# microsoft/StemGNN

Hardware: AMD Instinct MI355X
Metric: forecast-steps/sec (train) (higher is better)
Workload: dtype f32

## Files before the change

stemgnn_amd/csrc/gru.hip:

```cpp
#include <hip/hip_runtime.h>

#include "../../include/stemgnn_hip.h"
#include "gemm2.h"
#include "wgrad.h"
#include "dq_reduce.h"
#include "gemm_core.h"
#include "gru_wide.h"

#define SG_TRY(e)                                \
  do {                                           \
    hipError_t _e = (e);                         \
    if (_e != hipSuccess) return -(int)_e;       \
  } while (0)

__device__ __forceinline__ float gru_sigmoid(float v) { return 1.f / (1.f + expf(-v)); }
__device__ __forceinline__ int gru_uniform(int v) { return __builtin_amdgcn_readfirstlane(v); }

struct GruGiOp {
  const float *x, *w_ih, *b_ih;
  float* gi;
  int B, S, Hd, W;
  unsigned *za, *zb;
  unsigned na, nb;
  __device__ bool setup(int, int& M, int& N, int& K0, int& K1) const {
// ... 465 lines not shown
typedef float gru_f2 __attribute__((ext_vector_type(2)));
#ifndef GRU_NR_FWD
#define GRU_NR_FWD 8
#endif
#ifndef GRU_NR_BWD
#define GRU_NR_BWD 16
#endif
#ifndef GRU_NR4
#define GRU_NR4 16
#endif
#define GRU_NR2(P, OW) (((OW) == 1 && (P) <= 4) ? GRU_NR_BWD : 64)
#define GRU_NR3(KU) ((KU) <= 58 ? GRU_NR_FWD : 32)
template <int KU, int NR>
struct GruBcast {
  static constexpr int NRK = NR < KU ? (NR & ~3) : ((KU + 3) & ~3);
  static constexpr int NL = NRK < KU ? (KU - NRK + 3) / 4 : 0;
  float4 v[NL > 0 ? NL : 1];
  float hv;
  __device__ __forceinline__ GruBcast(float hv_, float* lrow, int lane) : hv(hv_) {
    if constexpr (NL > 0) {
      lrow[lane] = hv_;
      asm volatile("" ::: "memory");
#pragma unroll
      for (int i = 0; i < NL; ++i) v[i] = *reinterpret_cast<const float4*>(lrow + NRK + 4 * i);
      __builtin_amdgcn_sched_barrier(0);
    }
  }
  __device__ __forceinline__ gru_f2 pair(int kk) const {
    if (kk < NRK) return gru_f2{gru_bcast(hv, kk), gru_bcast(hv, kk + 1)};
    const float4 t = v[NL > 0 ? (kk - NRK) >> 2 : 0];
    return ((kk - NRK) & 2) ? gru_f2{t.z, t.w} : gru_f2{t.x, t.y};
  }
};
template <int KU, int NR>
__device__ __forceinline__ float gru_matvec(const gru_f2 (&wr)[32], float hv, float* lrow, int lane) {
  const GruBcast<KU, NR> bc(hv, lrow, lane);
  gru_f2 a0 = {0.f, 0.f}, a1 = {0.f, 0.f};
#pragma unroll
  for (int kk = 0; kk + 3 < KU; kk += 4) {
    a0 = __builtin_elementwise_fma(wr[kk >> 1], bc.pair(kk), a0);
    a1 = __builtin_elementwise_fma(wr[(kk >> 1) + 1], bc.pair(kk + 2), a1);
  }
  if constexpr ((KU & 3) != 0) a0 = __builtin_elementwise_fma(wr[(KU - 2) >> 1], bc.pair(KU - 2), a0);
  return (a0.x + a1.x) + (a0.y + a1.y);
}
__device__ __forceinline__ float gru_poll_lane(const gru_u64* g, unsigned tag, bool active, int* status) {
  float v = 0.f;
  if (active) v = gru_consume(g, tag, status);
  return v;
}

#ifdef GRU_PROF
#define GRU_T(var) const long long var = (long long)__builtin_readcyclecounter()
#define GRU_ACC(acc, t1, t0) acc += (t1) - (t0)
#else
#define GRU_T(var)
#define GRU_ACC(acc, t1, t0)
#endif
template <int KU, int NR>
__device__ __forceinline__ void gru_matvec3(const gru_f2 (&w0)[32], const gru_f2 (&w1)[32], const gru_f2 (&w2)[32],
                                            float hv, float* lrow, int lane, float& o0, float& o1, float& o2) {
  const GruBcast<KU, NR> bc(hv, lrow, lane);
  gru_f2 a0 = {0.f, 0.f}, b0 = {0.f, 0.f}, a1 = {0.f, 0.f}, b1 = {0.f, 0.f}, a2 = {0.f, 0.f}, b2 = {0.f, 0.f};
#pragma unroll
  for (int kk = 0; kk + 3 < KU; kk += 4) {
    const gru_f2 h0 = bc.pair(kk), h1 = bc.pair(kk + 2);
    a0 = __builtin_elementwise_fma(w0[kk >> 1], h0, a0);
    a1 = __builtin_elementwise_fma(w1[kk >> 1], h0, a1);
    a2 = __builtin_elementwise_fma(w2[kk >> 1], h0, a2);
    b0 = __builtin_elementwise_fma(w0[(kk >> 1) + 1], h1, b0);
    b1 = __builtin_elementwise_fma(w1[(kk >> 1) + 1], h1, b1);
    b2 = __builtin_elementwise_fma(w2[(kk >> 1) + 1], h1, b2);
  }
  if constexpr ((KU & 3) != 0) {
    const gru_f2 h0 = bc.pair(KU - 2);
    a0 = __builtin_elementwise_fma(w0[(KU - 2) >> 1], h0, a0);
    a1 = __builtin_elementwise_fma(w1[(KU - 2) >> 1], h0, a1);
    a2 = __builtin_elementwise_fma(w2[(KU - 2) >> 1], h0, a2);
  }
  o0 = (a0.x + b0.x) + (a0.y + b0.y);
  o1 = (a1.x + b1.x) + (a1.y + b1.y);
  o2 = (a2.x + b2.x) + (a2.y + b2.y);
}
template <int P, int KU, int OW>
__global__ __launch_bounds__(3 * (P / OW) * 64) void gru_bwd_cluster2_kernel(const float* __restrict__ dout, const float* __restrict__ w_hh,
                                                                      const float* __restrict__ h_all,
                                                                      const float* __restrict__ reserve, int B, int S, int Hd,
                                                                      gru_u64* __restrict__ xbuf, int* __restrict__ status,
                                                                      float* __restrict__ dgi, float* __restrict__ dghn,
                                                                      int s_hi, int s_lo, float* __restrict__ carry,
                                                                      int s_mark, unsigned* __restrict__ progress,
                                                                      gru_u64* __restrict__ xid, int allow_fast) {
  static_assert(P % OW == 0, "owners per wave");
  constexpr int NTH = 3 * (P / OW) * 64;
  __shared__ float part[2][3 * P][64];
  __shared__ __attribute__((aligned(16))) float lrow[3 * P][64];
  __shared__ int s_fast;
  int b, p;
  gru_cluster_ids(B, P, b, p);
  if (b >= B) return;
  const bool fast = P > 1 && gru_same_xcd(xid + (size_t)b * P, p, P, allow_fast, status, &s_fast, threadIdx.x);
  const int U = (Hd + P - 1) / P;
  const int tid = threadIdx.x, lane = tid & 63;
  const int wave = gru_uniform(tid >> 6);
  const int g = wave / (P / OW), q0 = (wave - g * (P / OW)) * OW;
  const int u0 = p * U, un = max(0, min(Hd, u0 + U) - u0);
  const int H3 = 3 * Hd;
  gru_f2 wr[OW][32];
  int k0[OW], kn[OW];
#pragma unroll
  for (int o = 0; o < OW; ++o) {
    k0[o] = ((q0 + o + p) % P) * U;
    kn[o] = max(0, min(Hd, k0[o] + U) - k0[o]);
    const bool lane_ok = lane < un;
    const float* wcol = w_hh + ((size_t)g * Hd + (kn[o] > 0 ? k0[o] : 0)) * Hd + (lane_ok ? u0 + lane : 0);
#pragma unroll
    for (int kk = 0; kk < KU; ++kk) {
      const float v = wcol[(size_t)(kk < kn[o] ? kk : 0) * Hd];
      wr[o][kk >> 1][kk & 1] = (lane_ok && kk < kn[o]) ? v : 0.f;
    }
  }
  const int gu = u0 + (tid < un ? tid : 0);
  float dhz = s_hi < S - 1 ? carry[(size_t)b * Hd + gu] : 0.f;
  for (int i = tid; i < 2 * 3 * P * 64; i += NTH) (&part[0][0][0])[i] = 0.f;
  size_t prow = (size_t)s_hi * B + b;
  float p_do = dout[prow * Hd + gu];
  float p_r = reserve[prow * 4 * Hd + gu], p_z = reserve[prow * 4 * Hd + Hd + gu];
  float p_n = reserve[prow * 4 * Hd + 2 * Hd + gu], p_g = reserve[prow * 4 * Hd + 3 * Hd + gu];
  float p_h = h_all[(s_hi > 0 ? prow - B : prow) * Hd + gu];
  __syncthreads();

#ifdef GRU_PROF
  long long c_poll = 0, c_mv = 0, c_bar = 0, c_gate = 0;
#endif
  for (int s = s_hi; s >= s_lo; --s) {
    const size_t row = (size_t)s * B + b;
    const unsigned tag = (unsigned)(S - s);
    gru_u64* xb = xbuf + ((size_t)(tag & 1) * B + b) * H3;
    float own_dr = 0.f;
    GRU_T(t0);
    if (tid < un) {
      float dh = p_do + dhz;
#pragma unroll
      for (int w = 0; w < 3 * P; ++w) dh += part[(tag + 1) & 1][w][tid];
      const float r = p_r, z = p_z, n = p_n, ghn = p_g;
      const float hprev = s > 0 ? p_h : 0.f;
      const float dn = dh * (1.f - z) * (1.f - n * n);
      const float dz = dh * (hprev - n) * z * (1.f - z);
      const float dr = dn * ghn * r * (1.f - r);
      const float dnr = dn * r;
      own_dr = dr;
      dhz = dh * z;
      if (s > 0) {
        gru_publish_x(xb + gu, tag, dr, fast);
        gru_publish_x(xb + Hd + gu, tag, dz, fast);
        gru_publish_x(xb + 2 * Hd + gu, tag, dnr, fast);
        const size_t rn = row - B;
        p_do = dout[rn * Hd + gu];
        p_r = reserve[rn * 4 * Hd + gu]; p_z = reserve[rn * 4 * Hd + Hd + gu];
        p_n = reserve[rn * 4 * Hd + 2 * Hd + gu]; p_g = reserve[rn * 4 * Hd + 3 * Hd + gu];
        p_h = h_all[(s > 1 ? rn - B : rn) * Hd + gu];
      }
      float* go = dgi + row * H3;
      go[gu] = dr; go[Hd + gu] = dz; go[2 * Hd + gu] = dn;
      dghn[row * Hd + gu] = dnr;
    }
// ... 250 lines not shown
    gru_hh_gemms(q, base, base + (size_t)3 * S * B * Hd, base, base, base, Hd);
    p.hh_form = gru_hh_form(q, Hd).form;
  }
  return p;
}
extern "C" int stemgnn_gru_paths(int B, int S, int Hd, int W, int cus, int* out) {
  if (B <= 0 || S <= 0 || Hd <= 0 || W <= 0 || !out) return SG_EINVAL;
  const GruPlan p = gru_plan(B, S, Hd, W, cus > 0 ? gru_limit_of_cus(cus) : gru_resident_limit());
  const bool wide = p.fwd_family == SG_GRU_FAM_WIDE;
  out[SG_GRU_FWD_FAMILY] = p.fwd_family; out[SG_GRU_FWD_P] = p.PF; out[SG_GRU_FWD_K] = p.KF;
  out[SG_GRU_GI_STREAM] = p.gi_stream;
  out[SG_GRU_BWD_FAMILY] = p.bwd_family; out[SG_GRU_BWD_P] = p.P; out[SG_GRU_BWD_KU] = p.KU;
  out[SG_GRU_BWD_SLICES] = p.slices; out[SG_GRU_IH_FOLDED] = p.fold_ih; out[SG_GRU_HH_FORM] = p.hh_form;
  out[SG_GRU_IH_SLABS] = p.ih_sum; out[SG_GRU_RANK2_OK] = p.rank2_ok;
  out[SG_GRU_WIDE_PASSES] = wide ? (B + GW_BP - 1) / GW_BP : 0;
  out[SG_GRU_WIDE_MT] = wide ? p.wide.MT : 0;
  out[SG_GRU_WIDE_GWF] = wide ? gru_wide_gwf_class(p.wide) : 0;
  out[SG_GRU_WIDE_GWB] = wide ? gru_wide_gwb_class(p.wide) : 0;
  return 0;
}

extern "C" size_t stemgnn_gru_fwd_scratch_floats(int B, int S, int Hd) {
  return (size_t)3 * Hd * Hd + (size_t)3 * S * B * Hd + gru_xbuf_floats(B, Hd) + 4;
}
static size_t gru_bwd_scratch_base(int B, int S, int Hd, int W) {
  return (size_t)4 * S * B * Hd + (size_t)GRU_NSPLIT * 3 * Hd * (Hd + 1) + (size_t)gru_ih_slabs(B) * 3 * Hd * (W + 1) +
         gru_xbuf_floats(B, Hd) + 4 + (size_t)B * Hd + 8 + 136;
}
constexpr size_t GRU_OVL_CLAIMS = 64 * 33;
static size_t gru_ovl_words(int S) { return (((size_t)S + 4 + GRU_OVL_CLAIMS + 64 + 8) + 3) & ~(size_t)3; }
extern "C" size_t stemgnn_gru_bwd_scratch_floats(int B, int S, int Hd, int W) {
  return ((gru_bwd_scratch_base(B, S, Hd, W) + 3) & ~(size_t)3) + gru_ovl_words(S);
}
extern "C" size_t stemgnn_gru_bwd_ctl_words(int S) { return S > 0 ? gru_ovl_words(S) + 64 : 0; }

extern "C" int stemgnn_gru_bwd_cus(int B, int Hd) {
  if (B <= 0 || Hd <= 0) return 0;
  const GruPlan pl = gru_plan(B, Hd, Hd, 1, gru_resident_limit());
  if (pl.bwd_family == SG_GRU_FAM_WIDE) return pl.wide.P;
  return B * (pl.P > 0 ? pl.P : 1);
}

template <bool RS>
static int gru_fwd_impl(const float* x, const float* w_ih, const float* w_hh, const float* b_ih, const float* b_hh, int B,
                        int S, int Hd, int W, float* scratch, float* h_ext, float* reserve, int* status, void* stream) {
  if (!x || !w_ih || !w_hh || !b_ih || !b_hh || !scratch || !h_ext || (RS && !reserve) || !status || B <= 0 || S <= 0 ||
      Hd <= 0 || W <= 0)
    return SG_EINVAL;
  hipStream_t st = (hipStream_t)stream;
  const GruPlan pl = gru_plan(B, S, Hd, W, gru_resident_limit());
  const bool use_wide = pl.fwd_family == SG_GRU_FAM_WIDE, use_c4 = pl.fwd_family == SG_GRU_FAM_CLUSTER4;
  float* h_all = h_ext + (size_t)B * Hd;
  float* w_hhT = scratch;
  float* gi = scratch + (size_t)3 * Hd * Hd;
  gru_u64* xbuf2 = (gru_u64*)(scratch + ((((size_t)3 * Hd * Hd + (size_t)3 * S * B * Hd) + 1) & ~(size_t)1));
  size_t zn0 = 0, zn1 = 0;
  if (use_c4) {
    zn0 = (size_t)B * Hd; zn1 = ((size_t)2 * B * Hd + (size_t)8 * B) * 2;
  } else {
    SG_TRY(sg_zero_async(h_ext, (size_t)B * Hd * sizeof(float), st));
  }
  if (pl.gi_stream && (reinterpret_cast<uintptr_t>(gi) & 15) == 0) {
    const int ncg = 3 * Hd / 4;
    hipLaunchKernelGGL(gru_gi_stream_kernel<12>, dim3((S * B + GI_RB - 1) / GI_RB, (ncg + GI_NT - 1) / GI_NT), dim3(GI_NT), 0,
                       st, x, w_ih, b_ih, gi, B, S, Hd, reinterpret_cast<unsigned*>(h_ext), reinterpret_cast<unsigned*>(xbuf2),
                       (unsigned)zn0, (unsigned)zn1);
    SG_TRY(hipGetLastError());
  } else {
    GruGiOp op{x, w_ih, b_ih, gi, B, S, Hd, W, reinterpret_cast<unsigned*>(h_ext), reinterpret_cast<unsigned*>(xbuf2),
               (unsigned)zn0, (unsigned)zn1};
    SG_TRY((sg_launch_gemm<GruGiOp, 64, 64, true, true, false>(op, S * B, 3 * Hd, 1, st)));
  }
  if (use_wide) {
    float* xb = scratch + ((((size_t)3 * Hd * Hd + (size_t)3 * S * B * Hd) + 3) & ~(size_t)3);
    SG_TRY(gru_wide_fwd<RS>(gi, w_hh, b_hh, B, S, Hd, pl.wide, xb, status, h_all, reserve, st));
    return 0;
  }
  if (use_c4) {
    gru_u64* xbuf = xbuf2;
    gru_u64* xid = xbuf + (size_t)2 * B * Hd;
    static const int allow_fast = !(getenv("STEMGNN_GRU_FAST_XCD") && atoi(getenv("STEMGNN_GRU_FAST_XCD")) == 0);
    const int PF = pl.PF, KF = pl.KF;
    const dim3 grid4(8 * ((B + 7) / 8) * PF);
#define GRU_F4K(PP, KK) hipLaunchKernelGGL((gru_fwd_cluster4_kernel<PP, KK, RS>), grid4, dim3((PP + 2) * 64), 0, st, gi, w_hh, \
                                           b_hh, B, S, Hd, xbuf, status, h_all, reserve, xid, allow_fast)
#define GRU_F4(PP) do { if (KF == 32) GRU_F4K(PP, 32); else if (KF == 34) GRU_F4K(PP, 34); else if (KF == 40) GRU_F4K(PP, 40); \
                        else if (KF == 48) GRU_F4K(PP, 48); else if (KF == 58) GRU_F4K(PP, 58); else GRU_F4K(PP, 64); } while (0)
    if (PF == 1) GRU_F4(1); else if (PF == 2) GRU_F4(2); else if (PF == 4) GRU_F4(4); else if (PF == 5) GRU_F4(5);
    else if (PF == 6) GRU_F4(6); else if (PF == 7) GRU_F4(7); else GRU_F4(8);
#undef GRU_F4
#undef GRU_F4K
    SG_TRY(hipGetLastError());
    return 0;
  }
  if (pl.fwd_family == SG_GRU_FAM_CLUSTER1) {
    const int P = pl.PF;
    const GruCluster c = gru_cluster_geom(Hd, P);
    gru_u64* xbuf = (gru_u64*)(scratch + ((((size_t)3 * Hd * Hd + (size_t)3 * S * B * Hd) + 1) & ~(size_t)1));
    if (P > 1) SG_TRY(sg_zero_async(xbuf, (size_t)2 * B * Hd * sizeof(gru_u64), st));
    const size_t lds = (size_t)(Hd + GRU_KC + c.ksf * 3 * c.U) * sizeof(float);
    const dim3 grid(8 * ((B + 7) / 8) * P);
    hipLaunchKernelGGL((gru_fwd_cluster_kernel<GRU_KC, RS>), grid, dim3(1024), lds, st, gi, w_hh, b_hh, B, S, Hd, P, xbuf,
                       status, h_all, reserve);
    SG_TRY(hipGetLastError());
    return 0;
  }
  hipLaunchKernelGGL(gru_transpose_kernel, dim3((Hd + 31) / 32, (3 * Hd + 31) / 32), dim3(256), 0, st, w_hh, w_hhT,
                     3 * Hd, Hd);
  SG_TRY(hipGetLastError());
  const int nub = (Hd + 63) / 64;
  const int ks = nub >= 16 ? 1 : 16 / nub;
  const size_t lds = (size_t)(Hd + ks * 3 * Hd) * sizeof(float);
  if (lds > 64 * 1024) return SG_EINVAL;
  hipLaunchKernelGGL(gru_fwd_kernel<RS>, dim3(B), dim3(1024), lds, st, gi, w_hhT, b_hh, B, S, Hd, h_all, reserve);
  SG_TRY(hipGetLastError());
  return 0;
}

extern "C" int stemgnn_gru_fwd(const float* x, const float* w_ih, const float* w_hh, const float* b_ih,
                               const float* b_hh, int B, int S, int Hd, int W, float* scratch, float* h_ext,
                               float* reserve, int* status, void* stream) {
  return gru_fwd_impl<true>(x, w_ih, w_hh, b_ih, b_hh, B, S, Hd, W, scratch, h_ext, reserve, status, stream);
}
extern "C" int stemgnn_gru_fwd_infer(const float* x, const float* w_ih, const float* w_hh, const float* b_ih,
                                     const float* b_hh, int B, int S, int Hd, int W, float* scratch, float* h_ext,
                                     int* status, void* stream) {
  return gru_fwd_impl<false>(x, w_ih, w_hh, b_ih, b_hh, B, S, Hd, W, scratch, h_ext, nullptr, status, stream);
}

static int gru_wgrad_rows(const float* dgi, const float* dghn, const float* h_ext, const float* x, float* p_hh, float* p_ih,
                          int B, int S, int Hd, int W, int row0, int rows, int slab0, int nsplit, hipStream_t st_hh,
                          hipStream_t st_ih, bool do_ih = true, bool do_hh = true) {
  const int chunk = ((rows + nsplit - 1) / nsplit + 15) & ~15;
  if (do_hh) {
    G2Args g;
    G2SlabEpi e;
    g.A[0] = dgi + (size_t)row0 * 3 * Hd;  g.lda[0] = 3 * Hd; g.M[0] = 2 * Hd;
    g.A[1] = dghn + (size_t)row0 * Hd;     g.lda[1] = Hd;     g.M[1] = Hd;
    for (int r = 0; r < 2; ++r) { g.B[r] = h_ext + (size_t)row0 * Hd; g.ldb[r] = Hd; g.N[r] = Hd + 1; g.K[r] = rows; }
    g.nsplit = nsplit; g.chunk = chunk; g.b_ones_col = Hd;
    e.part[0] = p_hh + (size_t)slab0 * 2 * Hd * (Hd + 1);
    e.part[1] = p_hh + (size_t)GRU_NSPLIT * 2 * Hd * (Hd + 1) + (size_t)slab0 * Hd * (Hd + 1);
    SG_TRY((g2_launch<G2SlabEpi, false, false>(g, e, 2, st_hh)));
  }
  if (!do_ih) return 0;
  GruWihGradOp o2{dgi, x, p_ih + (size_t)slab0 * 3 * Hd * (W + 1), B, S, Hd, W, nsplit, chunk, row0, rows};
  SG_TRY((sg_launch_gemm<GruWihGradOp, 64, 32, false, false, false, 64>(o2, 3 * Hd, W + 1, nsplit, st_ih)));
  return 0;
}
extern "C" int stemgnn_gru_bwd_rank2_ok(int B, int Hd) {
  if (B <= 0 || Hd <= 0) return 0;
  return gru_plan(B, Hd, Hd, 1, gru_resident_limit()).rank2_ok;
}
static int gru_bwd_impl(const float* dh_all, const float* dkey, const float* dquery, const float* wk, const float* wq,
                        const float* x, const float* w_hh, const float* h_ext, const float* reserve, int B, int S, int Hd,
                        int W, float* scratch, float* dw_ih, float* dw_hh, float* db_ih, float* db_hh, int* status,
                        void* stream, int stages = 3, void* side = nullptr, unsigned* ctl = nullptr, int dq_nchunk = 0,
                        int wg_split = 0, bool no_wgrad = false);
extern "C" int stemgnn_gru_bwd(const float* dh_all, const float* x, const float* w_hh, const float* h_ext,
                               const float* reserve, int B, int S, int Hd, int W, float* scratch, float* dw_ih,
                               float* dw_hh, float* db_ih, float* db_hh, int* status, void* stream) {
  if (!dh_all) return SG_EINVAL;
  return gru_bwd_impl(dh_all, nullptr, nullptr, nullptr, nullptr, x, w_hh, h_ext, reserve, B, S, Hd, W, scratch, dw_ih, dw_hh,
                      db_ih, db_hh, status, stream);
}
extern "C" int stemgnn_gru_bwd_rank2(const float* dkey, const float* dquery, const float* wk, const float* wq, const float* x,
                                     const float* w_hh, const float* h_ext, const float* reserve, int B, int S, int Hd, int W,
                                     float* scratch, float* dw_ih, float* dw_hh, float* db_ih, float* db_hh, int* status,
// ... 299 lines not shown
```

stemgnn_amd/csrc/gru_cluster4.h:

```cpp
#pragma once

#ifndef GRU_PUB_PUSH
#define GRU_PUB_PUSH 0
#endif
__device__ __forceinline__ void gru4_after_publish(const gru_u64* g) {
#if GRU_PUB_PUSH == 1
  asm volatile("s_waitcnt vmcnt(0)" ::: "memory");
#elif GRU_PUB_PUSH == 2
  gru_u64 x;
  asm volatile("global_load_dwordx2 %0, %1, off sc1" : "=v"(x) : "v"(g) : "memory");
  asm volatile("" :: "v"(x));
#else
  (void)g;
#endif
}
#ifndef GRU_POLL_MODE
#define GRU_POLL_MODE 0
#endif
#ifndef GRU_POLL_PRE_F
#define GRU_POLL_PRE_F 10
#endif
#ifndef GRU_POLL_PRE_B
#define GRU_POLL_PRE_B 9
#endif
#ifndef GRU_POLL_LOOP_SLEEP
#define GRU_POLL_LOOP_SLEEP 1
#endif
#include "gru_math.h"

template <int PRE>
__device__ __forceinline__ float gru4_poll(const gru_u64* g, unsigned tag, bool active, int* status) {
  if (PRE > 0) __builtin_amdgcn_s_sleep(PRE);
#if (GRU_POLL_MODE & 1)
  float v = 0.f;
  if (active) {
    gru_u64 a = __hip_atomic_load(g, __ATOMIC_RELAXED, __HIP_MEMORY_SCOPE_AGENT);
    __builtin_amdgcn_s_sleep(2);
    gru_u64 b = __hip_atomic_load(g, __ATOMIC_RELAXED, __HIP_MEMORY_SCOPE_AGENT);
    unsigned spins = 0;
    for (;;) {
      if ((unsigned)(a >> 32) == tag) { v = __uint_as_float((unsigned)a); break; }
      a = __hip_atomic_load(g, __ATOMIC_RELAXED, __HIP_MEMORY_SCOPE_AGENT);
      if ((unsigned)(b >> 32) == tag) { v = __uint_as_float((unsigned)b); break; }
      b = __hip_atomic_load(g, __ATOMIC_RELAXED, __HIP_MEMORY_SCOPE_AGENT);
      if (++spins > (1u << 22)) { atomicExch(status, 1); break; }
    }
  }
  return v;
#else
  float v = 0.f;
  if (active) {
    gru_u64 x = __hip_atomic_load(g, __ATOMIC_RELAXED, __HIP_MEMORY_SCOPE_AGENT);
    unsigned spins = 0;
    while ((unsigned)(x >> 32) != tag) {
      if (GRU_POLL_LOOP_SLEEP > 0) __builtin_amdgcn_s_sleep(GRU_POLL_LOOP_SLEEP);
      x = __hip_atomic_load(g, __ATOMIC_RELAXED, __HIP_MEMORY_SCOPE_AGENT);
      if (++spins > (1u << 22)) { atomicExch(status, 1); break; }
    }
    v = __uint_as_float((unsigned)x);
  }
  return v;
#endif
}
template <int PRE>
__device__ __forceinline__ void gru4_poll2(const gru_u64* g0, const gru_u64* g1, unsigned tag, bool act0, bool act1,
                                           int* status, float (&v)[2]) {
  if (PRE > 0) __builtin_amdgcn_s_sleep(PRE);
  gru_u64 x0 = __hip_atomic_load(g0, __ATOMIC_RELAXED, __HIP_MEMORY_SCOPE_AGENT);
  gru_u64 x1 = __hip_atomic_load(g1, __ATOMIC_RELAXED, __HIP_MEMORY_SCOPE_AGENT);
  unsigned spins = 0;
  while (act0 && (unsigned)(x0 >> 32) != tag) {
    if (GRU_POLL_LOOP_SLEEP > 0) __builtin_amdgcn_s_sleep(GRU_POLL_LOOP_SLEEP);
    x0 = __hip_atomic_load(g0, __ATOMIC_RELAXED, __HIP_MEMORY_SCOPE_AGENT);
    if (++spins > (1u << 22)) { atomicExch(status, 1); break; }
  }
  spins = 0;
  while (act1 && (unsigned)(x1 >> 32) != tag) {
    if (GRU_POLL_LOOP_SLEEP > 0) __builtin_amdgcn_s_sleep(GRU_POLL_LOOP_SLEEP);
    x1 = __hip_atomic_load(g1, __ATOMIC_RELAXED, __HIP_MEMORY_SCOPE_AGENT);
    if (++spins > (1u << 22)) { atomicExch(status, 1); break; }
  }
  v[0] = act0 ? __uint_as_float((unsigned)x0) : 0.f;
  v[1] = act1 ? __uint_as_float((unsigned)x1) : 0.f;
}
constexpr int gru4_static_lds_floats(int P, int nin, int nout) { return 2 * 3 * P * 64 + 3 * P * 64 + 2 * nin * 64 + 2 * nout * 64; }

constexpr int GRU4_WMAX = 16;
#ifndef GRU_CHORE_SLEEP_F
#define GRU_CHORE_SLEEP_F 20
#endif
#ifndef GRU_SW_MODE
#define GRU_SW_MODE 0
#endif
#ifndef GRU_SW_SLEEP
#define GRU_SW_SLEEP 30
#endif
#ifndef GRU_CHORE_SLEEP_B
#define GRU_CHORE_SLEEP_B 10
#endif
template <int P, int KU, bool RS = true>
__global__ __launch_bounds__((P + 2) * 64) void gru_fwd_cluster4_kernel(const float* __restrict__ gi, const float* __restrict__ w_hh,
                                                                        const float* __restrict__ b_hh, int B, int S, int Hd,
                                                                        gru_u64* __restrict__ xbuf, int* __restrict__ status,
                                                                        float* __restrict__ h_all, float* __restrict__ reserve,
                                                                        gru_u64* __restrict__ xid, int allow_fast) {
  __shared__ float part[2][3 * P][64];
  __shared__ __attribute__((aligned(16))) float lrow[P][64];
  __shared__ float gin[2][3][64];
  __shared__ float stash[2][5][64];
  __shared__ int s_fast;
  int b, p;
  gru_cluster_ids(B, P, b, p);
  if (b >= B) return;
  const bool fast = P > 1 && gru_same_xcd(xid + (size_t)b * P, p, P, allow_fast, status, &s_fast, threadIdx.x);
  const int U = (Hd + P - 1) / P;
  const int tid = threadIdx.x, lane = tid & 63;
  const int wave = gru_uniform(tid >> 6);
  const int u0 = p * U, un = max(0, min(Hd, u0 + U) - u0);
  const int H3 = 3 * Hd;
  const bool lane_ok = lane < un;
  const int gu = u0 + (lane_ok ? lane : 0);

  if (wave < P) {
    const int q = wave;
    const int k0 = ((q + p) % P) * U, kn = max(0, min(Hd, k0 + U) - k0);
    gru_f2 wr[3][32];
#pragma unroll
    for (int g = 0; g < 3; ++g) {
      const float* wrow = w_hh + ((size_t)g * Hd + gu) * Hd + (kn > 0 ? k0 : 0);
#pragma unroll
      for (int kk = 0; kk < KU; ++kk) {
        const float v = wrow[kk < kn ? kk : 0];
        wr[g][kk >> 1][kk & 1] = (lane_ok && kk < kn) ? v : 0.f;
      }
    }
    const gru_u64* pollp = xbuf + (size_t)b * Hd + k0 + (lane < kn ? lane : 0);
    const size_t par = (size_t)B * Hd;
#ifdef GRU_PROF
    long long c_a = 0, c_b = 0, c_c = 0;
#endif
    for (int s = 0; s < S; ++s) {
      GRU_T(t0);
      float hv = 0.f;
      if (s > 0) hv = gru4_poll<GRU_POLL_PRE_F>(pollp + (s & 1) * par, (unsigned)s, lane < kn, status);
      GRU_T(t1);
      GRU_ACC(c_a, t1, t0);
      float o0, o1, o2;
      gru_matvec3<KU, GRU_NR3(KU)>(wr[0], wr[1], wr[2], hv, lrow[q], lane, o0, o1, o2);
      part[s & 1][0 * P + q][lane] = o0;
      part[s & 1][1 * P + q][lane] = o1;
      part[s & 1][2 * P + q][lane] = o2;
      GRU_T(t2);
      GRU_ACC(c_b, t2, t1);
      gru_lds_barrier();
      GRU_T(t3);
      GRU_ACC(c_c, t3, t2);
    }
    gru_lds_barrier();
#ifdef GRU_PROF
    if (blockIdx.x == 0 && lane == 0)
      printf("gru fwd4 mat-vec wave %d: per step cycles: poll %lld  matvec %lld  barrier wait %lld\n", wave, c_a / S, c_b / S, c_c / S);
#endif
  } else if (wave == P + 1) {
    const float* gip = gi + (size_t)b * H3 + gu;
    const size_t grow = (size_t)B * H3;
    float v0 = gip[0], v1 = gip[Hd], v2 = gip[2 * Hd];
    for (int s = 0; s < S; ++s) {
      gin[s & 1][0][lane] = v0;
      gin[s & 1][1][lane] = v1;
      gin[s & 1][2][lane] = v2;
      float r = 0.f, z = 0.f, n = 0.f, g2 = 0.f, hn = 0.f;
      if (s >= 2) {
        r = stash[s & 1][0][lane]; z = stash[s & 1][1][lane]; n = stash[s & 1][2][lane];
        g2 = stash[s & 1][3][lane]; hn = stash[s & 1][4][lane];
      }
      if (s > 0) __builtin_amdgcn_s_sleep(GRU_CHORE_SLEEP_F);
      if (s + 1 < S) {
        const float* gn = gip + (size_t)(s + 1) * grow;
        v0 = gn[0]; v1 = gn[Hd]; v2 = gn[2 * Hd];
      }
      if (s >= 2 && lane_ok) {
        const size_t rw = (size_t)(s - 2) * B + b;
        if constexpr (RS) {
          float* rs = reserve + rw * 4 * Hd + gu;
          rs[0] = r; rs[Hd] = z; rs[2 * Hd] = n; rs[3 * Hd] = g2;
        }
        h_all[rw * Hd + gu] = hn;
      }
      gru_lds_barrier();
    }
    gru_lds_barrier();
    for (int t = (S >= 2 ? S - 2 : S - 1); t < S; ++t) {
      const size_t rw = (size_t)t * B + b;
      if (lane_ok) {
        if constexpr (RS) {
          float* rs = reserve + rw * 4 * Hd + gu;
          rs[0] = stash[t & 1][0][lane]; rs[Hd] = stash[t & 1][1][lane]; rs[2 * Hd] = stash[t & 1][2][lane];
          rs[3 * Hd] = stash[t & 1][3][lane];
        }
        h_all[rw * Hd + gu] = stash[t & 1][4][lane];
      }
    }
  } else {
    const float bh0 = b_hh[gu], bh1 = b_hh[Hd + gu], bh2 = b_hh[2 * Hd + gu];
    float hown = 0.f;
    gru_u64* pub = xbuf + (size_t)b * Hd + gu;
    const size_t par = (size_t)B * Hd;
#ifdef GRU_PROF
    long long c_a = 0, c_b = 0, c_c = 0;
#endif
    for (int s = 0; s < S; ++s) {
      GRU_T(t0);
      gru_lds_barrier();
      GRU_T(t1);
      GRU_ACC(c_a, t1, t0);
      float g0 = bh0, g1 = bh1, g2 = bh2;
#pragma unroll
      for (int qq = 0; qq < P; ++qq) {
        g0 += part[s & 1][0 * P + qq][lane];
        g1 += part[s & 1][1 * P + qq][lane];
        g2 += part[s & 1][2 * P + qq][lane];
      }
      const float gp0 = gin[s & 1][0][lane], gp1 = gin[s & 1][1][lane], gp2 = gin[s & 1][2][lane];
      const float r = gru4_sigmoid(gp0 + g0);
      const float z = gru4_sigmoid(gp1 + g1);
      const float n = gru4_tanh(gp2 + r * g2);
      const float hn = (1.f - z) * n + z * hown;
      hown = hn;
      if (s + 1 < S && lane_ok) gru_publish_x(pub + ((s + 1) & 1) * par, (unsigned)(s + 1), hn, fast);
      gru4_after_publish(pub);
      GRU_T(t2);
      GRU_ACC(c_b, t2, t1);
      stash[s & 1][0][lane] = r;
      stash[s & 1][1][lane] = z;
      stash[s & 1][2][lane] = n;
      stash[s & 1][3][lane] = g2;
      stash[s & 1][4][lane] = hn;
      GRU_T(t3);
      GRU_ACC(c_c, t3, t2);
    }
    gru_lds_barrier();
#ifdef GRU_PROF
    if (blockIdx.x == 0 && lane == 0)
      printf("gru fwd4 gate wave: per step cycles: barrier wait %lld  gate phase to publish %lld  stash %lld\n", c_a / S, c_b / S, c_c / S);
#endif
  }
}

template <int P, int KU, int OW = 1, bool SW = false>
__global__ __launch_bounds__((3 * P / OW + 2 + (SW ? 1 : 0)) * 64) void gru_bwd_cluster4_kernel(const float* __restrict__ dout, const float* __restrict__ w_hh,
                                                                            const float* __restrict__ h_all,
                                                                            const float* __restrict__ reserve, int B, int S, int Hd,
                                                                            gru_u64* __restrict__ xbuf, int* __restrict__ status,
                                                                            float* __restrict__ dgi, float* __restrict__ dghn,
                                                                            gru_u64* __restrict__ xid, int allow_fast,
                                                                            const float* __restrict__ x, float* __restrict__ ih_slab,
                                                                            int W, const float* __restrict__ dkey,
                                                                            const float* __restrict__ dquery,
                                                                            const float* __restrict__ wk, const float* __restrict__ wq,
                                                                            unsigned* __restrict__ prog, int prog_ts) {
  static_assert(P % OW == 0 && (OW == 1 || OW == 2), "owner slices per wave");
  constexpr int NMV = 3 * P / OW;
  __shared__ float part[2][NMV][64];
  __shared__ __attribute__((aligned(16))) float lrow[NMV][64];
  __shared__ float bin[2][6][64];
  __shared__ float bout[2][4][64];
  __shared__ int s_fast;
  int b, p;
  gru_cluster_ids(B, P, b, p);
  if (b >= B) return;
  const bool fast = P > 1 && gru_same_xcd(xid + (size_t)b * P, p, P, allow_fast, status, &s_fast, threadIdx.x);
  const int U = (Hd + P - 1) / P;
  const int tid = threadIdx.x, lane = tid & 63;
  const int wave = gru_uniform(tid >> 6);
  const int u0 = p * U, un = max(0, min(Hd, u0 + U) - u0);
  const int H3 = 3 * Hd;
  const bool lane_ok = lane < un;
  const int gu = u0 + (lane_ok ? lane : 0);
  for (int i = tid; i < 2 * NMV * 64; i += (int)blockDim.x) (&part[0][0][0])[i] = 0.f;

  if (wave < NMV) {
    const int g = wave / (P / OW), q0 = (wave - g * (P / OW)) * OW;
    gru_f2 wr[OW][32];
    int kn[OW];
    const gru_u64* pollp[OW];
#pragma unroll
    for (int o = 0; o < OW; ++o) {
      const int k0 = ((q0 + o + p) % P) * U;
      kn[o] = max(0, min(Hd, k0 + U) - k0);
      const float* wcol = w_hh + ((size_t)g * Hd + (kn[o] > 0 ? k0 : 0)) * Hd + gu;
#pragma unroll
      for (int kk = 0; kk < KU; ++kk) {
        const float v = wcol[(size_t)(kk < kn[o] ? kk : 0) * Hd];
        wr[o][kk >> 1][kk & 1] = (lane_ok && kk < kn[o]) ? v : 0.f;
      }
      pollp[o] = xbuf + (size_t)b * H3 + (size_t)g * Hd + k0 + (lane < kn[o] ? lane : 0);
    }
    const size_t par = (size_t)B * H3;
#ifdef GRU_PROF
    long long c_a = 0, c_b = 0, c_c = 0;
#endif
    gru_lds_barrier();
    for (int s = S - 1; s >= 1; --s) {
      const unsigned tag = (unsigned)(S - s);
      GRU_T(t0);
      float pv;
      if constexpr (OW == 1) {
        const float dv = gru4_poll<GRU_POLL_PRE_B>(pollp[0] + (tag & 1) * par, tag, lane < kn[0], status);
        pv = gru_matvec<KU, (KU <= 58 ? GRU_NR4 : (GRU_NR4 > 24 ? GRU_NR4 : 24))>(wr[0], dv, lrow[wave], lane);
      } else {
        float dv[2];
        gru4_poll2<GRU_POLL_PRE_B>(pollp[0] + (tag & 1) * par, pollp[1] + (tag & 1) * par, tag, lane < kn[0], lane < kn[1],
                                   status, dv);
        pv = gru_matvec<KU, 64>(wr[0], dv[0], lrow[wave], lane);
        pv += gru_matvec<KU, 64>(wr[OW - 1], dv[1], lrow[wave], lane);
      }
      part[tag & 1][wave][lane] = pv;
      GRU_T(t2);
      GRU_ACC(c_b, t2, t0);
      gru_lds_barrier();
      GRU_T(t3);
      GRU_ACC(c_c, t3, t2);
    }
    gru_lds_barrier();
#ifdef GRU_PROF
    if (blockIdx.x == 0 && lane == 0)
      printf("gru bwd4 mat-vec wave %d: per step cycles: poll %lld  matvec %lld  barrier wait %lld\n", wave, c_a / S, c_b / S, c_c / S);
#endif
  } else if (wave == NMV + 1) {
    const bool factored = dkey != nullptr;
    const float dk_own = factored ? dkey[(size_t)b * Hd + gu] : 0.f, dq_own = factored ? dquery[(size_t)b * Hd + gu] : 0.f;
    auto fetch = [&](int t, float (&val)[6]) {
      const size_t rw = (size_t)t * B + b;
      const float* rs = reserve + rw * 4 * Hd + gu;
      val[0] = factored ? dk_own * wk[t] + dq_own * wq[t] : dout[rw * Hd + gu];
      val[1] = rs[0]; val[2] = rs[Hd]; val[3] = rs[2 * Hd]; val[4] = rs[3 * Hd];
      val[5] = t > 0 ? h_all[(rw - B) * Hd + gu] : 0.f;
    };
    auto stage = [&](int t, const float (&val)[6]) {
#pragma unroll
      for (int v = 0; v < 6; ++v) bin[t & 1][v][lane] = val[v];
    };
    constexpr bool wt = SW;
    auto put = [&](size_t rw, float dr, float dz, float dn, float dnr) {
      if (wt) return;
      float* go = dgi + rw * H3 + gu;
      go[0] = dr; go[Hd] = dz; go[2 * Hd] = dn;
      dghn[rw * Hd + gu] = dnr;
    };
    auto flush = [&](int t) {
      const size_t rw = (size_t)t * B + b;
      const float dr = bout[t & 1][0][lane], dz = bout[t & 1][1][lane], dn = bout[t & 1][2][lane], dnr = bout[t & 1][3][lane];
      if (lane_ok) put(rw, dr, dz, dn, dnr);
    };
    float acc[3][GRU4_WMAX], accb[3] = {0.f, 0.f, 0.f};
#pragma unroll
    for (int g = 0; g < 3; ++g)
#pragma unroll
      for (int w = 0; w < GRU4_WMAX; ++w) acc[g][w] = 0.f;
    const float* xrow = x + (size_t)b * W * S;
    auto wih_x = [&](int t, float (&xv)[GRU4_WMAX]) {
      if (!ih_slab) return;
#pragma unroll
      for (int w = 0; w < GRU4_WMAX; ++w) xv[w] = xrow[(size_t)(w < W ? w : 0) * S + t];
    };
    auto wih = [&](const float (&xv)[GRU4_WMAX], float dr, float dz, float dn) {
      if (!ih_slab) return;
      accb[0] += dr; accb[1] += dz; accb[2] += dn;
#pragma unroll
      for (int w = 0; w < GRU4_WMAX; ++w) {
        acc[0][w] = fmaf(dr, xv[w], acc[0][w]);
        acc[1][w] = fmaf(dz, xv[w], acc[1][w]);
        acc[2][w] = fmaf(dn, xv[w], acc[2][w]);
      }
    };
    float val[6];
    fetch(S - 1, val);
    stage(S - 1, val);
    if (S >= 2) fetch(S - 2, val);
    gru_lds_barrier();
    for (int s = S - 1; s >= 1; --s) {
      stage(s - 1, val);
      float dr = 0.f, dz = 0.f, dn = 0.f, dnr = 0.f;
      const bool have = s + 1 <= S - 1;
      if (have) { dr = bout[(s + 1) & 1][0][lane]; dz = bout[(s + 1) & 1][1][lane]; dn = bout[(s + 1) & 1][2][lane]; dnr = bout[(s + 1) & 1][3][lane]; }
      float xv[GRU4_WMAX];
      if (have) wih_x(s + 1, xv);
      __builtin_amdgcn_s_sleep(GRU_CHORE_SLEEP_B);
      if (s >= 2) fetch(s - 2, val);
      if (have && lane_ok) put((size_t)(s + 1) * B + b, dr, dz, dn, dnr);
      if (have) wih(xv, dr, dz, dn);
      gru_lds_barrier();
    }
    gru_lds_barrier();
    float xv[GRU4_WMAX];
    if (S >= 2) { flush(1); wih_x(1, xv); wih(xv, bout[1][0][lane], bout[1][1][lane], bout[1][2][lane]); }
    flush(0);
    wih_x(0, xv);
    wih(xv, bout[0][0][lane], bout[0][1][lane], bout[0][2][lane]);
    if (ih_slab && lane_ok) {
#pragma unroll
      for (int g = 0; g < 3; ++g) {
        float* o = ih_slab + ((size_t)b * H3 + (size_t)g * Hd + gu) * (W + 1);
#pragma unroll
        for (int w = 0; w < GRU4_WMAX; ++w)
          if (w < W) o[w] = acc[g][w];
        o[W] = accb[g];
      }
    }
  } else if (SW && wave == NMV + 2) {
    auto put = [&](int t) {
      const size_t rw = (size_t)t * B + b;
      const float dr = bout[t & 1][0][lane], dz = bout[t & 1][1][lane], dn = bout[t & 1][2][lane], dnr = bout[t & 1][3][lane];
      if (lane_ok) {
        float* go = dgi + rw * H3 + gu;
#if GRU_SW_MODE == 0
        __hip_atomic_store(go, dr, __ATOMIC_RELAXED, __HIP_MEMORY_SCOPE_AGENT);
        __hip_atomic_store(go + Hd, dz, __ATOMIC_RELAXED, __HIP_MEMORY_SCOPE_AGENT);
        __hip_atomic_store(go + 2 * Hd, dn, __ATOMIC_RELAXED, __HIP_MEMORY_SCOPE_AGENT);
        __hip_atomic_store(dghn + rw * Hd + gu, dnr, __ATOMIC_RELAXED, __HIP_MEMORY_SCOPE_AGENT);
#elif GRU_SW_MODE == 2
        go[0] = dr; go[Hd] = dz; go[2 * Hd] = dn; dghn[rw * Hd + gu] = dnr;
#elif GRU_SW_MODE == 3
        __builtin_nontemporal_store(dr, go); __builtin_nontemporal_store(dz, go + Hd);
        __builtin_nontemporal_store(dn, go + 2 * Hd); __builtin_nontemporal_store(dnr, dghn + rw * Hd + gu);
#else
        if (dr + dz + dn + dnr == 1.2345e-30f) go[0] = dr;
#endif
      }
    };
    auto count = [&](int t) {
      if (lane == 0) __hip_atomic_fetch_add(prog + t / prog_ts, 1u, __ATOMIC_RELAXED, __HIP_MEMORY_SCOPE_AGENT);
    };
    gru_lds_barrier();
    for (int s = S - 1; s >= 1; --s) {
      __builtin_amdgcn_s_sleep(GRU_SW_SLEEP);
      if (s + 1 <= S - 1) put(s + 1);
      if (s + 3 <= S - 1 && (s + 3) % prog_ts == 0) {
        asm volatile("s_waitcnt vmcnt(8)" ::: "memory");
        count(s + 3);
      }
      gru_lds_barrier();
    }
    gru_lds_barrier();
    if (S >= 2) put(1);
    put(0);
    asm volatile("s_waitcnt vmcnt(0)" ::: "memory");
    for (int t = (S - 1 < 3 ? S - 1 : 3); t >= 0; --t)
      if (t % prog_ts == 0) count(t);
  } else {
    float dhz = 0.f;
    gru_u64* pub = xbuf + (size_t)b * H3 + gu;
    const size_t par = (size_t)B * H3;
#ifdef GRU_PROF
    long long c_a = 0, c_b = 0, c_c = 0;
#endif
    gru_lds_barrier();
    for (int s = S - 1; s >= 0; --s) {
      const unsigned tag = (unsigned)(S - s);
      GRU_T(t1);
      float dh = bin[s & 1][0][lane] + dhz;
#pragma unroll
      for (int w = 0; w < NMV; ++w) dh += part[(tag + 1) & 1][w][lane];
      const float r = bin[s & 1][1][lane], z = bin[s & 1][2][lane], n = bin[s & 1][3][lane], ghn = bin[s & 1][4][lane];
      const float hprev = s > 0 ? bin[s & 1][5][lane] : 0.f;
      const float dn = dh * (1.f - z) * (1.f - n * n);
      const float dz = dh * (hprev - n) * z * (1.f - z);
      const float dr = dn * ghn * r * (1.f - r);
      const float dnr = dn * r;
      dhz = dh * z;
      if (s > 0 && lane_ok) {
        gru_u64* xb = pub + (tag & 1) * par;
        gru_publish_x(xb, tag, dr, fast);
        gru_publish_x(xb + Hd, tag, dz, fast);
        gru_publish_x(xb + 2 * Hd, tag, dnr, fast);
      }
      gru4_after_publish(pub);
      GRU_T(t2);
      GRU_ACC(c_b, t2, t1);
      bout[s & 1][0][lane] = dr;
      bout[s & 1][1][lane] = dz;
      bout[s & 1][2][lane] = dn;
      bout[s & 1][3][lane] = dnr;
      GRU_T(t3);
      GRU_ACC(c_c, t3, t2);
      if (s > 0) gru_lds_barrier();
      GRU_T(t4);
      GRU_ACC(c_a, t4, t3);
    }
    gru_lds_barrier();
#ifdef GRU_PROF
    if (blockIdx.x == 0 && lane == 0)
      printf("gru bwd4 gate wave: per step cycles: barrier wait %lld  gate phase to publish %lld  stash %lld\n", c_a / S, c_b / S, c_c / S);
#endif
  }
}
```

Before: 86770.

## Pack GRU forward gate rows into two slots and vectorize LDS partial sums

For slice widths between 33 and 40 units, the forward cluster4 mat-vec now packs the three gate rows of a slice into two 64-lane row sets, so each wave runs two FMA chains instead of three. The partial-sum buffers are transposed to a row-major, odd-float4-stride layout so the owner wave can read its partials as float4 and sum them, in both the forward and backward kernels. It also requests a large dynamic LDS allocation to hold occupancy down, and adjusts the poll and chore sleep constants. The risks are that the row packing has complex indexing and that the large LDS request limits how many blocks fit per CU.

```diff
diff --git a/stemgnn_amd/csrc/gru.hip b/stemgnn_amd/csrc/gru.hip
--- a/stemgnn_amd/csrc/gru.hip
+++ b/stemgnn_amd/csrc/gru.hip
@@ -571,6 +571,29 @@
   o1 = (a1.x + b1.x) + (a1.y + b1.y);
   o2 = (a2.x + b2.x) + (a2.y + b2.y);
 }
+constexpr int GRU_PACK_KMAX = 40;
+template <int KU, int NR>
+__device__ __forceinline__ void gru_matvec2(const gru_f2 (&w0)[GRU_PACK_KMAX / 2], const gru_f2 (&w1)[GRU_PACK_KMAX / 2],
+                                            float hv, float* lrow, int lane, float& o0, float& o1) {
+  static_assert(KU <= GRU_PACK_KMAX && (KU & 1) == 0, "packed mat-vec: slices of at most 40 units");
+  const GruBcast<KU, NR> bc(hv, lrow, lane);
+  gru_f2 a0 = {0.f, 0.f}, b0 = {0.f, 0.f}, a1 = {0.f, 0.f}, b1 = {0.f, 0.f};
+#pragma unroll
+  for (int kk = 0; kk + 3 < KU; kk += 4) {
+    const gru_f2 h0 = bc.pair(kk), h1 = bc.pair(kk + 2);
+    a0 = __builtin_elementwise_fma(w0[kk >> 1], h0, a0);
+    a1 = __builtin_elementwise_fma(w1[kk >> 1], h0, a1);
+    b0 = __builtin_elementwise_fma(w0[(kk >> 1) + 1], h1, b0);
+    b1 = __builtin_elementwise_fma(w1[(kk >> 1) + 1], h1, b1);
+  }
+  if constexpr ((KU & 3) != 0) {
+    const gru_f2 h0 = bc.pair(KU - 2);
+    a0 = __builtin_elementwise_fma(w0[(KU - 2) >> 1], h0, a0);
+    a1 = __builtin_elementwise_fma(w1[(KU - 2) >> 1], h0, a1);
+  }
+  o0 = (a0.x + b0.x) + (a0.y + b0.y);
+  o1 = (a1.x + b1.x) + (a1.y + b1.y);
+}
 template <int P, int KU, int OW>
 __global__ __launch_bounds__(3 * (P / OW) * 64) void gru_bwd_cluster2_kernel(const float* __restrict__ dout, const float* __restrict__ w_hh,
                                                                       const float* __restrict__ h_all,
@@ -987,8 +1010,10 @@
     static const int allow_fast = !(getenv("STEMGNN_GRU_FAST_XCD") && atoi(getenv("STEMGNN_GRU_FAST_XCD")) == 0);
     const int PF = pl.PF, KF = pl.KF;
     const dim3 grid4(8 * ((B + 7) / 8) * PF);
-#define GRU_F4K(PP, KK) hipLaunchKernelGGL((gru_fwd_cluster4_kernel<PP, KK, RS>), grid4, dim3((PP + 2) * 64), 0, st, gi, w_hh, \
-                                           b_hh, B, S, Hd, xbuf, status, h_all, reserve, xid, allow_fast)
+#define GRU_F4K(PP, KK) do { const size_t hog = gru4_fwd_hog_bytes(PP, KK); \
+    if (hog) (void)hipFuncSetAttribute((const void*)gru_fwd_cluster4_kernel<PP, KK, RS>, hipFuncAttributeMaxDynamicSharedMemorySize, (int)hog); \
+    hipLaunchKernelGGL((gru_fwd_cluster4_kernel<PP, KK, RS>), grid4, dim3((PP + 2) * 64), hog, st, gi, w_hh, \
+                       b_hh, B, S, Hd, xbuf, status, h_all, reserve, xid, allow_fast); } while (0)
 #define GRU_F4(PP) do { if (KF == 32) GRU_F4K(PP, 32); else if (KF == 34) GRU_F4K(PP, 34); else if (KF == 40) GRU_F4K(PP, 40); \
                         else if (KF == 48) GRU_F4K(PP, 48); else if (KF == 58) GRU_F4K(PP, 58); else GRU_F4K(PP, 64); } while (0)
     if (PF == 1) GRU_F4(1); else if (PF == 2) GRU_F4(2); else if (PF == 4) GRU_F4(4); else if (PF == 5) GRU_F4(5);
diff --git a/stemgnn_amd/csrc/gru_cluster4.h b/stemgnn_amd/csrc/gru_cluster4.h
--- a/stemgnn_amd/csrc/gru_cluster4.h
+++ b/stemgnn_amd/csrc/gru_cluster4.h
@@ -18,7 +18,7 @@
 #define GRU_POLL_MODE 0
 #endif
 #ifndef GRU_POLL_PRE_F
-#define GRU_POLL_PRE_F 10
+#define GRU_POLL_PRE_F 9
 #endif
 #ifndef GRU_POLL_PRE_B
 #define GRU_POLL_PRE_B 9
@@ -83,11 +83,54 @@
   v[0] = act0 ? __uint_as_float((unsigned)x0) : 0.f;
   v[1] = act1 ? __uint_as_float((unsigned)x1) : 0.f;
 }
-constexpr int gru4_static_lds_floats(int P, int nin, int nout) { return 2 * 3 * P * 64 + 3 * P * 64 + 2 * nin * 64 + 2 * nout * 64; }
+#ifndef GRU_FWD_PACK
+#define GRU_FWD_PACK 1
+#endif
+#ifndef GRU_PART_VEC
+#define GRU_PART_VEC 1
+#endif
+constexpr int gru4_part_stride(int n) { return 4 * (((n + 3) / 4) | 1); }
+template <int ROWS, int N, int P = 0>
+struct Gru4Part {
+  static constexpr int PS = gru4_part_stride(N);
+  static constexpr int FLOATS = GRU_PART_VEC ? ROWS * PS : ROWS * N;
+  static __device__ __forceinline__ int at(int row, int q) {
+#if GRU_PART_VEC
+    return row * PS + q;
+#else
+    return P > 0 ? ((row >> 6) * P + q) * 64 + (row & 63) : q * ROWS + row;
+#endif
+  }
+  static __device__ __forceinline__ float sum(const float* part, int row, float acc) {
+#if GRU_PART_VEC
+    float4 v[PS / 4];
+#pragma unroll
+    for (int i = 0; i < (N + 3) / 4; ++i) v[i] = *reinterpret_cast<const float4*>(part + row * PS + 4 * i);
+#pragma unroll
+    for (int q = 0; q < N; ++q) {
+      const float4 t = v[q >> 2];
+      acc += (q & 3) == 0 ? t.x : ((q & 3) == 1 ? t.y : ((q & 3) == 2 ? t.z : t.w));
+    }
+#else
+#pragma unroll
+    for (int q = 0; q < N; ++q) acc += part[at(row, q)];
+#endif
+    return acc;
+  }
+};
+constexpr int gru4_static_lds_floats(int P, int nin, int nout) {
+  return 2 * 64 * (GRU_PART_VEC ? gru4_part_stride(3 * P) : 3 * P) + 3 * P * 64 + 2 * nin * 64 + 2 * nout * 64;
+}
 
+constexpr bool gru4_fwd_packs(int KU) { return GRU_FWD_PACK != 0 && KU > 32 && KU <= 40; }
+constexpr size_t gru4_fwd_hog_bytes(int P, int KU) {
+  return gru4_fwd_packs(KU)
+             ? (size_t)156 * 1024 - sizeof(float) * (2 * 128 * (GRU_PART_VEC ? gru4_part_stride(P) : P) + P * 64 + 2 * 3 * 64 + 2 * 5 * 64)
+             : 0;
+}
 constexpr int GRU4_WMAX = 16;
 #ifndef GRU_CHORE_SLEEP_F
-#define GRU_CHORE_SLEEP_F 20
+#define GRU_CHORE_SLEEP_F 16
 #endif
 #ifndef GRU_SW_MODE
 #define GRU_SW_MODE 0
@@ -104,7 +147,9 @@
                                                                         gru_u64* __restrict__ xbuf, int* __restrict__ status,
                                                                         float* __restrict__ h_all, float* __restrict__ reserve,
                                                                         gru_u64* __restrict__ xid, int allow_fast) {
-  __shared__ float part[2][3 * P][64];
+  constexpr bool PACK = gru4_fwd_packs(KU);
+  typedef Gru4Part<PACK ? 128 : 192, P, PACK ? 0 : P> Part;
+  __shared__ __attribute__((aligned(16))) float part[2][Part::FLOATS];
   __shared__ __attribute__((aligned(16))) float lrow[P][64];
   __shared__ float gin[2][3][64];
   __shared__ float stash[2][5][64];
@@ -120,18 +165,34 @@
   const int H3 = 3 * Hd;
   const bool lane_ok = lane < un;
   const int gu = u0 + (lane_ok ? lane : 0);
+  if (un == 0) return;
 
   if (wave < P) {
     const int q = wave;
     const int k0 = ((q + p) % P) * U, kn = max(0, min(Hd, k0 + U) - k0);
     gru_f2 wr[3][32];
-#pragma unroll
-    for (int g = 0; g < 3; ++g) {
-      const float* wrow = w_hh + ((size_t)g * Hd + gu) * Hd + (kn > 0 ? k0 : 0);
-#pragma unroll
-      for (int kk = 0; kk < KU; ++kk) {
-        const float v = wrow[kk < kn ? kk : 0];
-        wr[g][kk >> 1][kk & 1] = (lane_ok && kk < kn) ? v : 0.f;
+    gru_f2 wp[2][GRU_PACK_KMAX / 2];
+    if constexpr (PACK) {
+#pragma unroll
+      for (int t = 0; t < 2; ++t) {
+        const int o = 64 * t + lane, g = o / U, u = o - g * U;
+        const bool live = o < 3 * U && u < un;
+        const float* wrow = w_hh + (live ? ((size_t)g * Hd + u0 + u) * Hd : (size_t)0) + (kn > 0 ? k0 : 0);
+#pragma unroll
+        for (int kk = 0; kk < KU; ++kk) {
+          const float v = wrow[kk < kn ? kk : 0];
+          wp[t][kk >> 1][kk & 1] = (live && kk < kn) ? v : 0.f;
+        }
+      }
+    } else {
+#pragma unroll
+      for (int g = 0; g < 3; ++g) {
+        const float* wrow = w_hh + ((size_t)g * Hd + gu) * Hd + (kn > 0 ? k0 : 0);
+#pragma unroll
+        for (int kk = 0; kk < KU; ++kk) {
+          const float v = wrow[kk < kn ? kk : 0];
+          wr[g][kk >> 1][kk & 1] = (lane_ok && kk < kn) ? v : 0.f;
+        }
       }
     }
     const gru_u64* pollp = xbuf + (size_t)b * Hd + k0 + (lane < kn ? lane : 0);
@@ -145,11 +206,19 @@
       if (s > 0) hv = gru4_poll<GRU_POLL_PRE_F>(pollp + (s & 1) * par, (unsigned)s, lane < kn, status);
       GRU_T(t1);
       GRU_ACC(c_a, t1, t0);
-      float o0, o1, o2;
-      gru_matvec3<KU, GRU_NR3(KU)>(wr[0], wr[1], wr[2], hv, lrow[q], lane, o0, o1, o2);
-      part[s & 1][0 * P + q][lane] = o0;
-      part[s & 1][1 * P + q][lane] = o1;
-      part[s & 1][2 * P + q][lane] = o2;
+      float* pw = part[s & 1];
+      if constexpr (PACK) {
+        float o0, o1;
+        gru_matvec2<KU, GRU_NR3(KU)>(wp[0], wp[1], hv, lrow[q], lane, o0, o1);
+        pw[Part::at(lane, q)] = o0;
+        pw[Part::at(64 + lane, q)] = o1;
+      } else {
+        float o0, o1, o2;
+        gru_matvec3<KU, GRU_NR3(KU)>(wr[0], wr[1], wr[2], hv, lrow[q], lane, o0, o1, o2);
+        pw[Part::at(lane, q)] = o0;
+        pw[Part::at(64 + lane, q)] = o1;
+        pw[Part::at(128 + lane, q)] = o2;
+      }
       GRU_T(t2);
       GRU_ACC(c_b, t2, t1);
       gru_lds_barrier();
@@ -204,6 +273,7 @@
   } else {
     const float bh0 = b_hh[gu], bh1 = b_hh[Hd + gu], bh2 = b_hh[2 * Hd + gu];
     float hown = 0.f;
+    const int row0 = PACK ? (lane < U ? lane : 0) : lane, rstep = PACK ? U : 64;
     gru_u64* pub = xbuf + (size_t)b * Hd + gu;
     const size_t par = (size_t)B * Hd;
 #ifdef GRU_PROF
@@ -214,13 +284,8 @@
       gru_lds_barrier();
       GRU_T(t1);
       GRU_ACC(c_a, t1, t0);
-      float g0 = bh0, g1 = bh1, g2 = bh2;
-#pragma unroll
-      for (int qq = 0; qq < P; ++qq) {
-        g0 += part[s & 1][0 * P + qq][lane];
-        g1 += part[s & 1][1 * P + qq][lane];
-        g2 += part[s & 1][2 * P + qq][lane];
-      }
+      const float* pr = part[s & 1];
+      const float g0 = Part::sum(pr, row0, bh0), g1 = Part::sum(pr, row0 + rstep, bh1), g2 = Part::sum(pr, row0 + 2 * rstep, bh2);
       const float gp0 = gin[s & 1][0][lane], gp1 = gin[s & 1][1][lane], gp2 = gin[s & 1][2][lane];
       const float r = gru4_sigmoid(gp0 + g0);
       const float z = gru4_sigmoid(gp1 + g1);
@@ -261,7 +326,8 @@
                                                                             unsigned* __restrict__ prog, int prog_ts) {
   static_assert(P % OW == 0 && (OW == 1 || OW == 2), "owner slices per wave");
   constexpr int NMV = 3 * P / OW;
-  __shared__ float part[2][NMV][64];
+  typedef Gru4Part<64, NMV> Part;
+  __shared__ __attribute__((aligned(16))) float part[2][Part::FLOATS];
   __shared__ __attribute__((aligned(16))) float lrow[NMV][64];
   __shared__ float bin[2][6][64];
   __shared__ float bout[2][4][64];
@@ -277,7 +343,7 @@
   const int H3 = 3 * Hd;
   const bool lane_ok = lane < un;
   const int gu = u0 + (lane_ok ? lane : 0);
-  for (int i = tid; i < 2 * NMV * 64; i += (int)blockDim.x) (&part[0][0][0])[i] = 0.f;
+  for (int i = tid; i < 2 * Part::FLOATS; i += (int)blockDim.x) (&part[0][0])[i] = 0.f;
 
   if (wave < NMV) {
     const int g = wave / (P / OW), q0 = (wave - g * (P / OW)) * OW;
@@ -315,7 +381,7 @@
         pv = gru_matvec<KU, 64>(wr[0], dv[0], lrow[wave], lane);
         pv += gru_matvec<KU, 64>(wr[OW - 1], dv[1], lrow[wave], lane);
       }
-      part[tag & 1][wave][lane] = pv;
+      part[tag & 1][Part::at(lane, wave)] = pv;
       GRU_T(t2);
       GRU_ACC(c_b, t2, t0);
       gru_lds_barrier();
@@ -459,9 +525,7 @@
     for (int s = S - 1; s >= 0; --s) {
       const unsigned tag = (unsigned)(S - s);
       GRU_T(t1);
-      float dh = bin[s & 1][0][lane] + dhz;
-#pragma unroll
-      for (int w = 0; w < NMV; ++w) dh += part[(tag + 1) & 1][w][lane];
+      const float dh = Part::sum(part[(tag + 1) & 1], lane, bin[s & 1][0][lane] + dhz);
       const float r = bin[s & 1][1][lane], z = bin[s & 1][2][lane], n = bin[s & 1][3][lane], ghn = bin[s & 1][4][lane];
       const float hprev = s > 0 ? bin[s & 1][5][lane] : 0.f;
       const float dn = dh * (1.f - z) * (1.f - n * n);
```

Result: faster. 87980, median of 6 (+1.4%).
